# pawanjay176/kzg_rust

Hardware: AMD Instinct MI355X
Metric: blobs/sec on verify_blob_kzg_proof_batch (mainnet 4096, batch=64) (higher is better)
Workload: dtype u32 limbs (29-bit) / 64-bit accumulate, u8 bytes

## Files before the change

__graft_entry__.py:

```python
import os
import subprocess
import sys

ROOT = os.path.dirname(os.path.abspath(__file__))
if ROOT not in sys.path:
    sys.path.insert(0, ROOT)


def build() -> None:
    env = dict(os.environ)
    subprocess.run(["make", "-C", os.path.join(ROOT, "kzg_rust_amd", "csrc"), "-j5"], check=True, env=env)
    subprocess.run(["make", "-C", os.path.join(ROOT, "oracle")], check=True, env=env)
    native = os.path.join(ROOT, "tests", "native")
    subprocess.run(["g++", "-O2", "-shared", "-fPIC", "-o", os.path.join(native, "libhd_probe.so"), os.path.join(native, "hd_probe.cpp")],
                   check=True, env=env)
    subprocess.run(["g++", "-O2", "-shared", "-fPIC", "-o", os.path.join(native, "liblazy_chain_probe.so"), os.path.join(native, "lazy_chain_probe.cpp")],
                   check=True, env=env)
    subprocess.run(["g++", "-O2", "-shared", "-fPIC", "-o", os.path.join(native, "libmont_columns_probe.so"), os.path.join(native, "mont_columns_probe.cpp")],
                   check=True, env=env)
    subprocess.run(["g++", "-std=c++17", "-O2", "-o", os.path.join(native, "cpp_vector_runner"), os.path.join(native, "cpp_vector_runner.cpp"),
                    "-L" + os.path.join(ROOT, "kzg_rust_amd"), "-lkzg355", "-Wl,-rpath," + os.path.join(ROOT, "kzg_rust_amd")], check=True, env=env)
    subprocess.run(["g++", "-std=c++17", "-O2", "-o", os.path.join(native, "cpp_cell_runner"), os.path.join(native, "cpp_cell_runner.cpp"),
                    "-L" + os.path.join(ROOT, "kzg_rust_amd"), "-lkzg355", "-Wl,-rpath," + os.path.join(ROOT, "kzg_rust_amd")], check=True, env=env)
    subprocess.run(["g++", "-std=c++17", "-O2", "-o", os.path.join(native, "cpp_cell_compute_runner"), os.path.join(native, "cpp_cell_compute_runner.cpp"),
                    "-L" + os.path.join(ROOT, "kzg_rust_amd"), "-lkzg355", "-Wl,-rpath," + os.path.join(ROOT, "kzg_rust_amd")], check=True, env=env)
    subprocess.run(["g++", "-std=c++17", "-O2", "-o", os.path.join(native, "cpp_cell_recover_runner"), os.path.join(native, "cpp_cell_recover_runner.cpp"),
                    "-L" + os.path.join(ROOT, "kzg_rust_amd"), "-lkzg355", "-Wl,-rpath," + os.path.join(ROOT, "kzg_rust_amd")], check=True, env=env)
    subprocess.run(["g++", "-std=c++17", "-O2", "-o", os.path.join(native, "cpp_cell_recover_sets_runner"), os.path.join(native, "cpp_cell_recover_sets_runner.cpp"),
                    "-L" + os.path.join(ROOT, "kzg_rust_amd"), "-lkzg355", "-Wl,-rpath," + os.path.join(ROOT, "kzg_rust_amd")], check=True, env=env)
    quad_src, quad_bin = os.path.join(native, "quad_ops_test.hip"), os.path.join(native, "quad_ops_test")
    quad_deps = [quad_src] + [os.path.join(ROOT, "kzg_rust_amd", "csrc", f) for f in ("g1_quad.h", "g1.h", "field.h", "modinv.h", "consts_gen.h")]
    if not os.path.exists(quad_bin) or any(os.path.getmtime(d) > os.path.getmtime(quad_bin) for d in quad_deps):
        subprocess.run(["/opt/rocm/bin/hipcc", "-O3", "-std=c++17", "--offload-arch=gfx950", "-Wno-unused-result", "-o", quad_bin, quad_src], check=True, env=env)
    probe_src, probe_so = os.path.join(native, "gpu_probe.hip"), os.path.join(native, "libgpu_probe.so")
    probe_deps = [probe_src] + [os.path.join(ROOT, "kzg_rust_amd", "csrc", f) for f in ("field.h", "modinv.h", "eval_core.h", "consts_gen.h")]
    if not os.path.exists(probe_so) or any(os.path.getmtime(d) > os.path.getmtime(probe_so) for d in probe_deps):
        subprocess.run(["/opt/rocm/bin/hipcc", "-O3", "-std=c++17", "--offload-arch=gfx950", "-Wno-unused-result", "-shared", "-fPIC", "-o", probe_so, probe_src],
                       check=True, env=env)
    group_src, group_so = os.path.join(native, "gpu_group_probe.hip"), os.path.join(native, "libgpu_group_probe.so")
    group_deps = [group_src] + [os.path.join(ROOT, "kzg_rust_amd", "csrc", f) for f in
                                ("field.h", "modinv.h", "tower.h", "g1.h", "pairing.h", "pairing_coop.h", "pairing_lanes.h", "consts_gen.h")]
    if not os.path.exists(group_so) or any(os.path.getmtime(d) > os.path.getmtime(group_so) for d in group_deps):
        subprocess.run(["/opt/rocm/bin/hipcc", "-O3", "-std=c++17", "--offload-arch=gfx950", "-Wno-unused-result", "-shared", "-fPIC", "-o", group_so, group_src],
                       check=True, env=env)
    import kzg_rust_amd
    from kzg_rust_amd import _lib
    lib = _lib.load()
    for name in _lib.EXPORTED_SYMBOLS:
        getattr(lib, name)
    print("build ok:", lib.kzg355_version().decode())


def smoke() -> None:
    import torch
    assert torch.cuda.is_available(), "smoke() needs a GPU"
    import kzg_rust_amd as kz
    from oracle.oracle import Oracle
    sys.path.insert(0, os.path.join(ROOT, "tests"))
    from synth import random_blob
    golden = os.path.join(ROOT, "tests", "golden")
    g1 = open(os.path.join(golden, "trusted_setup_g1.bin"), "rb").read()
    g2 = open(os.path.join(golden, "trusted_setup_g2.bin"), "rb").read()
    s = kz.Kzg.load_trusted_setup([g1[48 * i:48 * i + 48] for i in range(4096)], [g2[96 * i:96 * i + 96] for i in range(65)])
    o = Oracle()
    os_ = o.load_trusted_setup(g1, g2)
    blobs = [random_blob(1000 + i) for i in range(3)]
    cs = [kz.Kzg.blob_to_kzg_commitment(kz.Blob(b), s) for b in blobs]
    assert [c.to_bytes() for c in cs] == [o.blob_to_kzg_commitment(b, os_) for b in blobs], "commitment mismatch vs oracle"
    ps = [kz.Kzg.compute_blob_kzg_proof(kz.Blob(b), c, s) for b, c in zip(blobs, cs)]
    assert [p.to_bytes() for p in ps] == [o.compute_blob_kzg_proof(b, c.to_bytes(), os_) for b, c in zip(blobs, cs)], "proof mismatch vs oracle"
    ok = kz.Kzg.verify_blob_kzg_proof_batch([kz.Blob(b) for b in blobs], cs, ps, s)
    assert ok is True and o.verify_blob_kzg_proof_batch(blobs, [c.to_bytes() for c in cs], [p.to_bytes() for p in ps], os_) is True
    bad = [ps[1], ps[0], ps[2]]
    assert kz.Kzg.verify_blob_kzg_proof_batch([kz.Blob(b) for b in blobs], cs, bad, s) is False
    s.free()
    o.free_trusted_setup(os_)
    print("smoke ok: commit/prove bit-exact vs oracle, verify batch true/false as expected")


if __name__ == "__main__":
    build()
    if len(sys.argv) > 1 and sys.argv[1] == "smoke":
        smoke()
```

kzg_rust_amd/csrc/eval_core.h:

```cpp
#pragma once
#include "field.h"

namespace kzg {

struct EvalGroup { Fr sa, sb, st; };
constexpr int EVAL_ZPOWERS = 12;
constexpr int EVAL_WAVES = 4;
constexpr int EVAL_TAB_L1 = 0, EVAL_TAB_L2 = 1024, EVAL_TAB_L3 = 1280, EVAL_TAB_L4 = 1344, EVAL_TAB_L5 = 1360, EVAL_TAB_L6 = 1364, EVAL_TAB_GROUPS = 1365;
struct EvalPiece { uint32_t w[4]; };
constexpr int EVAL_TAB_PIECES = ((EVAL_TAB_GROUPS + 63) / 64) * 7 * 64;
KZG_HD constexpr int eval_tab_piece(int e, int q) { return (e / 64) * 7 * 64 + q * 64 + (e % 64); }
KZG_HD void eval_group_pack(EvalPiece p[7], const EvalGroup &g) {
    for (int k = 0; k < 28; k++) p[k / 4].w[k % 4] = k < NFR ? g.sa.l[k] : k < 2 * NFR ? g.sb.l[k - NFR] : k < 3 * NFR ? g.st.l[k - 2 * NFR] : 0u;
}
KZG_HD void eval_group_unpack(EvalGroup &g, const EvalPiece p[7]) {
#pragma unroll
    for (int k = 0; k < 27; k++) (k < NFR ? g.sa.l[k] : k < 2 * NFR ? g.sb.l[k - NFR] : g.st.l[k - 2 * NFR]) = p[k / 4].w[k % 4];
}
KZG_HD constexpr int eval_tab_first(int level) {
    return level == 1 ? EVAL_TAB_L1 : level == 2 ? EVAL_TAB_L2 : level == 3 ? EVAL_TAB_L3 : level == 4 ? EVAL_TAB_L4 : level == 5 ? EVAL_TAB_L5 : EVAL_TAB_L6;
}

template <int K> struct FrMultiple {
    uint32_t l[NFR];
    constexpr FrMultiple() : l{} {
        const uint32_t m[NFR] = FR_MOD_INIT;
        uint64_t c = 0;
        for (int i = 0; i < NFR; i++) { c += (uint64_t)m[i] * (uint32_t)K; l[i] = i < NFR - 1 ? (uint32_t)(c & LMASK) : (uint32_t)c; c >>= LB; }
    }
};
template <int K> KZG_HD void fr_sub_bias(Fr &r, const Fr &a, const Fr &b) {
    constexpr FrMultiple<K> kr;
    int32_t c = 0;
#pragma unroll
    for (int i = 0; i < NFR; i++) {
        const int32_t t = (int32_t)a.l[i] - (int32_t)b.l[i] + (int32_t)kr.l[i] + c;
        if (i < NFR - 1) { c = t >> LB; r.l[i] = (uint32_t)t & LMASK; }
        else r.l[i] = (uint32_t)t;
    }
}

KZG_HD void fr_add_raw(Fr &r, const Fr &a, const Fr &b) {
#pragma unroll
    for (int i = 0; i < NFR; i++) r.l[i] = a.l[i] + b.l[i];
}
template <int K> struct FrMultipleRaw {
    uint32_t l[NFR];
    constexpr FrMultipleRaw() : l{} {
        const FrMultiple<K> n;
        for (int i = 0; i < NFR; i++) l[i] = n.l[i] + (i < NFR - 1 ? (1u << LB) : 0u) - (i > 0 ? 1u : 0u);
    }
};
template <int K> KZG_HD void fr_sub_bias_raw(Fr &r, const Fr &a, const Fr &b) {
    constexpr FrMultipleRaw<K> kr;
#pragma unroll
    for (int i = 0; i < NFR; i++) r.l[i] = a.l[i] - b.l[i] + kr.l[i];
}
KZG_HD void fr_add_sweep(Fr &r, const Fr &a, const Fr &b) {
    uint32_t c = 0;
#pragma unroll
    for (int i = 0; i < NFR; i++) {
        const uint32_t t = a.l[i] + b.l[i] + c;
        if (i < NFR - 1) { c = t >> LB; r.l[i] = t & LMASK; } else r.l[i] = t;
    }
}

template <int K> KZG_HD void eval_node2(Fr &n, const Fr &n0, const Fr &n1, const Fr &zk, const Fr &s) {
    Fr A, B;
    fr_add_raw(A, n0, n1);
    fr_sub_bias_raw<K>(B, n0, n1);
    fr_mul2_lazy(n, A, zk, B, s);
}
KZG_HD void eval_group(Fr &n, const Fr c[4], const Fr &zk, const Fr &zk2, const EvalGroup &g) {
    Fr na, nb;
    eval_node2<2>(na, c[0], c[1], zk, g.sa);
    eval_node2<2>(nb, c[2], c[3], zk, g.sb);
    eval_node2<2>(n, na, nb, zk2, g.st);
}
KZG_HD void eval_group_leaves(Fr &n, Fr &Sp, const uint32_t pw[4][8], const Fr &z, const Fr &z2, const EvalGroup &g) {
    Fr p0, p1, p2, p3, A, B, na, nb, S;
    words_to_limbs<NFR, 8>(p0.l, pw[0]); words_to_limbs<NFR, 8>(p1.l, pw[1]);
    words_to_limbs<NFR, 8>(p2.l, pw[2]); words_to_limbs<NFR, 8>(p3.l, pw[3]);
    fr_add_raw(A, p0, p1); fr_sub_bias_raw<3>(B, p0, p1);
    fr_mul2_lazy(na, A, z, B, g.sa);
    fr_add_raw(S, p2, p3); fr_sub_bias_raw<3>(B, p2, p3);
    fr_mul2_lazy(nb, S, z, B, g.sb);
    fr_add_raw(S, S, A);
    fr_add_sweep(Sp, Sp, S);
    eval_node2<2>(n, na, nb, z2, g.st);
}
KZG_HD void eval_fold(Fr &s) { Fr t; fr_mul_lazy(t, s, fr_one()); s = t; }
KZG_HD void eval_finish(Fr &y, const Fr &ntop, const Fr &Sp, const Fr &z, const Fr &zN) {
    const uint32_t inv4096[NFR] = FR_INV4096_INIT;
    Fr k4096; for (int i = 0; i < NFR; i++) k4096.l[i] = inv4096[i];
    Fr negD, t;
    fr_sub(negD, fr_one(), zN);
    fr_mul2_lazy(t, ntop, z, Sp, negD);
    fr_mul(y, t, k4096);
}

}
```

kzg_rust_amd/csrc/k_verify.hip:

```cpp
#define KZG_FP_MUL_NOINLINE 1
#define KZG_MONT_COLS_FR 1
#include "kernels.h"
#include "sha256_rounds.h"
#include "fr_block.h"

namespace kzg {



constexpr int CH_BLOCKS = 2050;
struct ChallengeReader {
    const uint4 *blob; const uint8_t *cm;
    uint4 line[8];
    uint32_t carry[8];
    __device__ __forceinline__ void prefetch(int b) {
        if (b < 2048 && !(b & 1)) {
            const uint4 *p = blob + 4 * b;
#pragma unroll
            for (int q = 0; q < 8; q++) line[q] = p[q];
        }
    }
    __device__ __forceinline__ void words(uint32_t w[16], int b) {
        if (b == 0) {
            w[0] = 0x4653424cu; w[1] = 0x4f425645u; w[2] = 0x52494659u; w[3] = 0x5f56315fu;
            w[4] = 0; w[5] = 0; w[6] = 0; w[7] = (uint32_t)N_FE;
        } else if (b <= 2048) {
#pragma unroll
            for (int k = 0; k < 8; k++) w[k] = carry[k];
        }
        if (b < 2048) {
            uint4 s0, s1, s2, s3;
            if (b & 1) { s0 = line[4]; s1 = line[5]; s2 = line[6]; s3 = line[7]; }
            else { s0 = line[0]; s1 = line[1]; s2 = line[2]; s3 = line[3]; }
            w[8] = bswap32(s0.x); w[9] = bswap32(s0.y); w[10] = bswap32(s0.z); w[11] = bswap32(s0.w);
            w[12] = bswap32(s1.x); w[13] = bswap32(s1.y); w[14] = bswap32(s1.z); w[15] = bswap32(s1.w);
            carry[0] = bswap32(s2.x); carry[1] = bswap32(s2.y); carry[2] = bswap32(s2.z); carry[3] = bswap32(s2.w);
            carry[4] = bswap32(s3.x); carry[5] = bswap32(s3.y); carry[6] = bswap32(s3.z); carry[7] = bswap32(s3.w);
        } else if (b == 2048) {
            for (int k = 0; k < 8; k++) w[8 + k] = load_be32(cm + 4 * k);
        } else {
            for (int k = 0; k < 4; k++) w[k] = load_be32(cm + 32 + 4 * k);
            w[4] = 0x80000000u;
            for (int k = 5; k < 15; k++) w[k] = 0;
            w[15] = (uint32_t)((32 + BLOB_BYTES + 48) * 8);
        }
    }
};

__device__ __forceinline__ void challenge_finish(const uint32_t hh[8], int i, const uint8_t *cm, const uint8_t *proofs, Fr *z_out, Fr *zpow_out,
        uint8_t *records) {
    const uint32_t dw[8] = {hh[7], hh[6], hh[5], hh[4], hh[3], hh[2], hh[1], hh[0]};
    Fr z; fr_from_words(z, dw);
    z_out[i] = z;
    if (zpow_out) {
        Fr p = z;
#pragma unroll 1
        for (int k = 0; k < EVAL_ZPOWERS; k++) { fr_sqr(p, p); zpow_out[EVAL_ZPOWERS * (size_t)i + k] = p; }
    }
    if (!records) return;
    uint8_t *rec = records + (size_t)RECORD_BYTES * i;
    for (int k = 0; k < 48; k++) rec[k] = cm[k];
    uint8_t zb[32]; fr_to_be32(zb, z);
    for (int k = 0; k < 32; k++) rec[48 + k] = zb[k];
    const uint8_t *pr = proofs + 48 * (size_t)i;
    for (int k = 0; k < 48; k++) rec[112 + k] = pr[k];
}

__global__ void __launch_bounds__(128) k_challenge(const uint8_t *blobs, const uint8_t *commitments, const uint8_t *proofs, int n_total,
                                                    Fr *z_out, Fr *zpow_out, uint8_t *records) {
    __shared__ uint4 wk[2][16][64];
    const int lane = threadIdx.x & 63, role = threadIdx.x >> 6;
    const int i_raw = blockIdx.x * 64 + lane;
    const int i = i_raw < n_total ? i_raw : n_total - 1;
    const uint4 *blob = reinterpret_cast<const uint4 *>(blobs + (size_t)BLOB_BYTES * i);
    const uint8_t *cm = commitments + 48 * (size_t)i;
    static const uint32_t K[64] = {
        0x428a2f98u, 0x71374491u, 0xb5c0fbcfu, 0xe9b5dba5u, 0x3956c25bu, 0x59f111f1u, 0x923f82a4u, 0xab1c5ed5u,
        0xd807aa98u, 0x12835b01u, 0x243185beu, 0x550c7dc3u, 0x72be5d74u, 0x80deb1feu, 0x9bdc06a7u, 0xc19bf174u,
        0xe49b69c1u, 0xefbe4786u, 0x0fc19dc6u, 0x240ca1ccu, 0x2de92c6fu, 0x4a7484aau, 0x5cb0a9dcu, 0x76f988dau,
        0x983e5152u, 0xa831c66du, 0xb00327c8u, 0xbf597fc7u, 0xc6e00bf3u, 0xd5a79147u, 0x06ca6351u, 0x14292967u,
        0x27b70a85u, 0x2e1b2138u, 0x4d2c6dfcu, 0x53380d13u, 0x650a7354u, 0x766a0abbu, 0x81c2c92eu, 0x92722c85u,
        0xa2bfe8a1u, 0xa81a664bu, 0xc24b8b70u, 0xc76c51a3u, 0xd192e819u, 0xd6990624u, 0xf40e3585u, 0x106aa070u,
        0x19a4c116u, 0x1e376c08u, 0x2748774cu, 0x34b0bcb5u, 0x391c0cb3u, 0x4ed8aa4au, 0x5b9cca4fu, 0x682e6ff3u,
        0x748f82eeu, 0x78a5636fu, 0x84c87814u, 0x8cc70208u, 0x90befffau, 0xa4506cebu, 0xbef9a3f7u, 0xc67178f2u};
    ChallengeReader rd; rd.blob = blob; rd.cm = cm;
    auto produce = [&](int b) {
        uint32_t w[16];
        rd.words(w, b);
        rd.prefetch(b + 1);
        uint4 *dst = &wk[b & 1][0][lane];
#pragma unroll
        for (int t = 0; t < 64; t += 4) {
#pragma unroll
            for (int u = 0; u < 4; u++) {
                const int tt = t + u;
                if (tt >= 16) {
                    const uint32_t w15 = w[(tt + 1) & 15], w2 = w[(tt + 14) & 15];
                    const uint32_t s0 = xor3(ror(w15, 7), ror(w15, 18), w15 >> 3);
                    const uint32_t s1 = xor3(ror(w2, 17), ror(w2, 19), w2 >> 10);
                    w[tt & 15] = w[tt & 15] + s0 + w[(tt + 9) & 15] + s1;
                }
            }
            dst[(t >> 2) * 64] = make_uint4(w[t & 15] + K[t], w[(t + 1) & 15] + K[t + 1], w[(t + 2) & 15] + K[t + 2], w[(t + 3) & 15] + K[t + 3]);
        }
    };
    uint32_t h0 = 0x6a09e667u, h1 = 0xbb67ae85u, h2 = 0x3c6ef372u, h3 = 0xa54ff53au, h4 = 0x510e527fu, h5 = 0x9b05688cu, h6 = 0x1f83d9abu, h7 = 0x5be0cd19u;
    if (role == 1) { rd.prefetch(0); produce(0); }
    __syncthreads();
    for (int b = 0; b < CH_BLOCKS; b++) {
        if (role == 0) {
            uint32_t a = h0, bb = h1, c = h2, d = h3, e = h4, f = h5, g = h6, h = h7;
            const uint4 *src = &wk[b & 1][0][lane];
#pragma unroll
            for (int t = 0; t < 64; t += 4) {
                const uint4 q = src[(t >> 2) * 64];
                const uint32_t wv[4] = {q.x, q.y, q.z, q.w};
#pragma unroll
                for (int u = 0; u < 4; u++) {
                    const uint32_t t1 = h + xor3(ror(e, 6), ror(e, 11), ror(e, 25)) + ch3(e, f, g) + wv[u];
                    const uint32_t t2 = xor3(ror(a, 2), ror(a, 13), ror(a, 22)) + maj3(a, bb, c);
                    h = g; g = f; f = e; e = d + t1; d = c; c = bb; bb = a; a = t1 + t2;
                }
            }
            h0 += a; h1 += bb; h2 += c; h3 += d; h4 += e; h5 += f; h6 += g; h7 += h;
        } else if (b + 1 < CH_BLOCKS) {
            produce(b + 1);
        }
        __syncthreads();
    }
    if (role != 0 || i_raw >= n_total) return;
    const uint32_t hh[8] = {h0, h1, h2, h3, h4, h5, h6, h7};
    challenge_finish(hh, i, cm, proofs, z_out, zpow_out, records);
}

constexpr int CH1W_THREADS = 256;
__global__ void __launch_bounds__(CH1W_THREADS) k_challenge_1w(const uint8_t *blobs, const uint8_t *commitments, const uint8_t *proofs, int n_total,
                                                      Fr *z_out, Fr *zpow_out, uint8_t *records) {
    const int i_raw = blockIdx.x * CH1W_THREADS + threadIdx.x;
    const int i = i_raw < n_total ? i_raw : n_total - 1;
    const uint4 *blob = reinterpret_cast<const uint4 *>(blobs + (size_t)BLOB_BYTES * i);
    const uint8_t *cm = commitments + 48 * (size_t)i;
    static const uint32_t K[64] = {
        0x428a2f98u, 0x71374491u, 0xb5c0fbcfu, 0xe9b5dba5u, 0x3956c25bu, 0x59f111f1u, 0x923f82a4u, 0xab1c5ed5u,
        0xd807aa98u, 0x12835b01u, 0x243185beu, 0x550c7dc3u, 0x72be5d74u, 0x80deb1feu, 0x9bdc06a7u, 0xc19bf174u,
        0xe49b69c1u, 0xefbe4786u, 0x0fc19dc6u, 0x240ca1ccu, 0x2de92c6fu, 0x4a7484aau, 0x5cb0a9dcu, 0x76f988dau,
        0x983e5152u, 0xa831c66du, 0xb00327c8u, 0xbf597fc7u, 0xc6e00bf3u, 0xd5a79147u, 0x06ca6351u, 0x14292967u,
        0x27b70a85u, 0x2e1b2138u, 0x4d2c6dfcu, 0x53380d13u, 0x650a7354u, 0x766a0abbu, 0x81c2c92eu, 0x92722c85u,
        0xa2bfe8a1u, 0xa81a664bu, 0xc24b8b70u, 0xc76c51a3u, 0xd192e819u, 0xd6990624u, 0xf40e3585u, 0x106aa070u,
        0x19a4c116u, 0x1e376c08u, 0x2748774cu, 0x34b0bcb5u, 0x391c0cb3u, 0x4ed8aa4au, 0x5b9cca4fu, 0x682e6ff3u,
        0x748f82eeu, 0x78a5636fu, 0x84c87814u, 0x8cc70208u, 0x90befffau, 0xa4506cebu, 0xbef9a3f7u, 0xc67178f2u};
    uint32_t hh[8] = {0x6a09e667u, 0xbb67ae85u, 0x3c6ef372u, 0xa54ff53au, 0x510e527fu, 0x9b05688cu, 0x1f83d9abu, 0x5be0cd19u};
    ChallengeReader rd; rd.blob = blob; rd.cm = cm;
    rd.prefetch(0);
#pragma unroll 1
    for (int b = 0; b < CH_BLOCKS; b++) {
        uint32_t w[16];
        rd.words(w, b);
        rd.prefetch(b + 1);
        uint32_t a = hh[0], bb = hh[1], c = hh[2], d = hh[3], e = hh[4], f = hh[5], g = hh[6], h = hh[7];
#pragma unroll
        for (int t = 0; t < 64; t++) {
            if (t >= 16) {
                const uint32_t w15 = w[(t + 1) & 15], w2 = w[(t + 14) & 15];
                const uint32_t s0 = xor3(ror(w15, 7), ror(w15, 18), w15 >> 3);
                const uint32_t s1 = xor3(ror(w2, 17), ror(w2, 19), w2 >> 10);
                w[t & 15] = w[t & 15] + s0 + w[(t + 9) & 15] + s1;
            }
            const uint32_t t1 = h + xor3(ror(e, 6), ror(e, 11), ror(e, 25)) + ch3(e, f, g) + (w[t & 15] + K[t]);
            const uint32_t t2 = xor3(ror(a, 2), ror(a, 13), ror(a, 22)) + maj3(a, bb, c);
            h = g; g = f; f = e; e = d + t1; d = c; c = bb; bb = a; a = t1 + t2;
        }
        hh[0] += a; hh[1] += bb; hh[2] += c; hh[3] += d; hh[4] += e; hh[5] += f; hh[6] += g; hh[7] += h;
    }
    if (i_raw >= n_total) return;
    challenge_finish(hh, i, cm, proofs, z_out, zpow_out, records);
}

__global__ void __launch_bounds__(64) k_challenge_from_digest(const uint8_t *digests, const uint8_t *commitments, const uint8_t *proofs, int n_total,
                                                              Fr *z_out, Fr *zpow_out, uint8_t *records) {
    const int i = blockIdx.x * 64 + threadIdx.x;
    if (i >= n_total) return;
    uint32_t hh[8];
#pragma unroll
    for (int k = 0; k < 8; k++) hh[k] = load_be32(digests + 32 * (size_t)i + 4 * k);
    challenge_finish(hh, i, commitments + 48 * (size_t)i, proofs, z_out, zpow_out, records);
}

__device__ __forceinline__ void eval_issue_tile_loads(const uint4 *blob_step, uint4 *tile, int lane) {
#pragma unroll
    for (int q = 0; q < 8; q++) {
        const int g = 8 * q + (lane >> 3), s = lane & 7;
        __builtin_amdgcn_global_load_lds((const void __attribute__((address_space(1))) *)(blob_step + 8 * g + (s ^ (g & 7))),
                                         (void __attribute__((address_space(3))) *)(tile + 64 * q), 16, 0, 0);
    }
}
__device__ __forceinline__ void eval_tab_load(EvalPiece p[7], const EvalPiece *tab, int e) {
    const uint4 *src = reinterpret_cast<const uint4 *>(tab);
#pragma unroll
    for (int q = 0; q < 7; q++) { const uint4 v = src[eval_tab_piece(e, q)]; p[q].w[0] = v.x; p[q].w[1] = v.y; p[q].w[2] = v.z; p[q].w[3] = v.w; }
}
__device__ __forceinline__ void eval_park(uint32_t *hx, int entry, const Fr &h) {
#pragma unroll
    for (int k = 0; k < NFR; k++) hx[NFR * entry + k] = h.l[k];
}
__device__ __forceinline__ void eval_children(Fr c[4], const uint32_t *hx, int node) {
    __builtin_amdgcn_fence(__ATOMIC_RELEASE, "workgroup"); __builtin_amdgcn_wave_barrier(); __builtin_amdgcn_fence(__ATOMIC_ACQUIRE, "workgroup");
    const uint4 *src = reinterpret_cast<const uint4 *>(hx + 4 * NFR * node);
    uint32_t w[4 * NFR];
#pragma unroll
    for (int q = 0; q < NFR; q++) { const uint4 v = src[q]; w[4 * q] = v.x; w[4 * q + 1] = v.y; w[4 * q + 2] = v.z; w[4 * q + 3] = v.w; }
#pragma unroll
    for (int e = 0; e < 4; e++)
#pragma unroll
        for (int k = 0; k < NFR; k++) c[e].l[k] = w[NFR * e + k];
    __builtin_amdgcn_fence(__ATOMIC_RELEASE, "workgroup"); __builtin_amdgcn_wave_barrier();
}
__global__ void __launch_bounds__(64 * EVAL_WAVES, 2) k_eval(const uint8_t *blobs, const Fr *z_in, const Fr *zpow, const EvalPiece *tab, int n_total,
                                                          int n_per_group, Fr *y_out, uint8_t *records, int *err) {
    __shared__ uint4 tiles[EVAL_WAVES][512];
    __shared__ __attribute__((aligned(16))) uint32_t hxs[EVAL_WAVES][256 * NFR];
    const int wid = __builtin_amdgcn_readfirstlane((int)(threadIdx.x >> 6)), lane = threadIdx.x & 63;
    const int blob_raw = blockIdx.x * EVAL_WAVES + wid;
    const int blob_i = blob_raw < n_total ? blob_raw : n_total - 1;
    uint4 *tile = tiles[wid];
    uint32_t *hx = hxs[wid];
    const uint4 *blob = reinterpret_cast<const uint4 *>(blobs + (size_t)BLOB_BYTES * blob_i);
    eval_issue_tile_loads(blob, tile, lane);
    const Fr z = z_in[blob_i];
    const Fr *zp = zpow + EVAL_ZPOWERS * (size_t)blob_i;
    const Fr z2 = zp[0];
    __shared__ uint32_t zls[EVAL_WAVES][4 * NFR];
    const uint32_t zl_word = reinterpret_cast<const uint32_t *>(zp + 1)[lane < 4 * NFR ? lane : 0];
    Fr h2[4], Sp = fr_zero();
    bool bad = false;
    constexpr int STEPS = N_FE / 4 / 64;
    EvalPiece g_next[7];
    eval_tab_load(g_next, tab, EVAL_TAB_L1 + lane);
#pragma unroll 1
    for (int it = 0; it < STEPS; it++) {
        __builtin_amdgcn_s_waitcnt(0);
        __builtin_amdgcn_fence(__ATOMIC_ACQUIRE, "workgroup");
        if (it == 0 && lane < 4 * NFR) zls[wid][lane] = zl_word;
        uint4 cur[8];
#pragma unroll
        for (int j = 0; j < 8; j++) cur[j] = tile[8 * lane + (j ^ (lane & 7))];
        EvalGroup g1; eval_group_unpack(g1, g_next);
        __builtin_amdgcn_fence(__ATOMIC_RELEASE, "workgroup"); __builtin_amdgcn_wave_barrier();
        if (it + 1 < STEPS) eval_issue_tile_loads(blob + 512 * (it + 1), tile, lane);
        const int e_l1 = EVAL_TAB_L1 + ((it + 1) & (STEPS - 1)) * 64 + lane, e_l2 = EVAL_TAB_L2 + 64 * (it >> 2) + lane;
        eval_tab_load(g_next, tab, (it & 3) == 3 ? e_l2 : e_l1);
        uint32_t pw[4][8];
#pragma unroll
        for (int e = 0; e < 4; e++) {
            const uint4 a = cur[2 * e], b = cur[2 * e + 1];
            pw[e][7] = bswap32(a.x); pw[e][6] = bswap32(a.y); pw[e][5] = bswap32(a.z); pw[e][4] = bswap32(a.w);
            pw[e][3] = bswap32(b.x); pw[e][2] = bswap32(b.y); pw[e][1] = bswap32(b.z); pw[e][0] = bswap32(b.w);
        }
        const uint32_t top = max(max(pw[0][7], pw[1][7]), max(pw[2][7], pw[3][7]));
        if (top >= FR_MOD_TOP_WORD) {
#pragma unroll 1
            for (int e = 0; e < 4; e++) bad = bad || !fr_words_canonical(pw[e]);
        }
        Fr h;
        eval_group_leaves(h, Sp, pw, z, z2, g1);
        eval_park(hx, 64 * (it & 3) + lane, h);
        if ((it & 3) == 3) {
            Fr c[4];
            eval_children(c, hx, lane);
            EvalGroup g2; eval_group_unpack(g2, g_next);
            eval_tab_load(g_next, tab, it + 1 < STEPS ? e_l1 : EVAL_TAB_L3 + lane);
            Fr z4, z8;
#pragma unroll
            for (int k = 0; k < NFR; k++) { z4.l[k] = zls[wid][k]; z8.l[k] = zls[wid][NFR + k]; }
            Fr r2; eval_group(r2, c, z4, z8, g2);
#pragma unroll
            for (int a = 0; a < 4; a++) if ((it >> 2) == a) h2[a] = r2;
        }
    }
    if (bad && blob_raw < n_total) atomicOr(&err[blob_i / n_per_group], ERR_NONCANONICAL_FR);
    Fr c[4], h;
#pragma unroll
    for (int a = 0; a < 4; a++) eval_park(hx, 64 * a + lane, h2[a]);
    eval_children(c, hx, lane);
    EvalGroup g3; eval_group_unpack(g3, g_next);
    Fr z16, z32;
#pragma unroll
    for (int k = 0; k < NFR; k++) { z16.l[k] = zls[wid][2 * NFR + k]; z32.l[k] = zls[wid][3 * NFR + k]; }
    eval_group(h, c, z16, z32, g3);
    const int b = lane >> 4, u = lane & 15;
    const int mine_raw = blockIdx.x * EVAL_WAVES + b, mine = mine_raw < n_total ? mine_raw : n_total - 1;
    const Fr *zq = zpow + EVAL_ZPOWERS * (size_t)mine;
    Fr zt[7];
#pragma unroll
    for (int k = 0; k < 7; k++) zt[k] = zq[5 + k];
    const Fr zmine = z_in[mine];
    EvalPiece gp4[7], gp5[7], gp6[7];
    eval_tab_load(gp4, tab, EVAL_TAB_L4 + u); eval_tab_load(gp5, tab, EVAL_TAB_L5 + (lane & 3)); eval_tab_load(gp6, tab, EVAL_TAB_L6);
    eval_fold(Sp);
#pragma unroll
    for (int off = 32; off > 0; off >>= 1) { const Fr o = fr_shfl_down(Sp, off); fr_add_lazy(Sp, Sp, o); }
    eval_park(hx, lane, h);
    if (lane == 0) eval_park(hx, 64, Sp);
    __syncthreads();
    if (wid != 0) return;
    Fr Sb;
#pragma unroll
    for (int k = 0; k < NFR; k++) Sb.l[k] = hxs[b][NFR * 64 + k];
    eval_children(c, hxs[b], u);
    EvalGroup gt; eval_group_unpack(gt, gp4);
    eval_group(h, c, zt[0], zt[1], gt);
    uint32_t *hx0 = hxs[0];
    eval_park(hx0, lane, h);
    eval_children(c, hx0, 4 * b + (lane & 3));
    eval_group_unpack(gt, gp5);
    eval_group(h, c, zt[2], zt[3], gt);
    if (u < 4) eval_park(hx0, 4 * b + u, h);
    eval_children(c, hx0, b);
    eval_group_unpack(gt, gp6);
    eval_group(h, c, zt[4], zt[5], gt);
    Fr y; eval_finish(y, h, Sb, zmine, zt[6]);
    if (u == 0 && mine_raw < n_total) {
        if (records) {
            uint32_t yw[8]; limbs_to_words<NFR, 8>(yw, y.l);
            uint8_t *rec = records + (size_t)RECORD_BYTES * mine + 80;
#pragma unroll
            for (int i = 0; i < 8; i++) {
                const uint32_t v = yw[7 - i];
                rec[4 * i] = (uint8_t)(v >> 24); rec[4 * i + 1] = (uint8_t)(v >> 16); rec[4 * i + 2] = (uint8_t)(v >> 8); rec[4 * i + 3] = (uint8_t)v;
            }
        }
        if (y_out) {
            const uint32_t r2[NFR] = FR_R2_INIT;
            Fr R2; for (int i = 0; i < NFR; i++) R2.l[i] = r2[i];
            Fr ym; fr_mul(ym, y, R2);
            y_out[mine] = ym;
        }
    }
}

__global__ void __launch_bounds__(64) k_rhash_lanes(const uint8_t *records, int n, int groups, uint32_t *digests, int n_fe) {
    const int g = blockIdx.x * 64 + threadIdx.x;
    if (g >= groups) return;
    const uint8_t *rec = records + (size_t)RECORD_BYTES * n * g;
    const uint32_t total_words = 8u + 40u * (uint32_t)n;
    const uint32_t nblocks = (total_words * 4u + 9u + 63u) / 64u;
    const uint64_t bits = (uint64_t)total_words * 32u;
    uint32_t hs[8] = {0x6a09e667u, 0xbb67ae85u, 0x3c6ef372u, 0xa54ff53au, 0x510e527fu, 0x9b05688cu, 0x1f83d9abu, 0x5be0cd19u};
#pragma unroll 1
    for (uint32_t b = 0; b < nblocks; b++) {
        uint32_t w[16];
        if (b >= 1u && 16u * b + 16u <= total_words) {
            const uint4 *p = reinterpret_cast<const uint4 *>(rec + 64u * (size_t)b - 32u);
#pragma unroll
            for (int q = 0; q < 4; q++) {
                const uint4 v = p[q];
                w[4 * q] = bswap32(v.x); w[4 * q + 1] = bswap32(v.y); w[4 * q + 2] = bswap32(v.z); w[4 * q + 3] = bswap32(v.w);
            }
        } else {
#pragma unroll
            for (int t = 0; t < 16; t++) {
                const uint32_t idx = 16u * b + (uint32_t)t;
                uint32_t v;
                if (idx < 8u) {
                    const uint32_t hdr[8] = {0x52434b5au, 0x47424154u, 0x43485f5fu, 0x5f56315fu, 0u, (uint32_t)n_fe, 0u, (uint32_t)n};
                    v = hdr[idx];
                } else if (idx < total_words) v = bswap32(reinterpret_cast<const uint32_t *>(rec)[idx - 8u]);
                else if (idx == total_words) v = 0x80000000u;
                else if (idx == 16u * nblocks - 2u) v = (uint32_t)(bits >> 32);
                else if (idx == 16u * nblocks - 1u) v = (uint32_t)bits;
                else v = 0u;
                w[t] = v;
            }
        }
        uint32_t a = hs[0], bb = hs[1], c = hs[2], d = hs[3], e = hs[4], f = hs[5], gg = hs[6], h = hs[7];
#pragma unroll
        for (int t = 0; t < 64; t++) {
            if (t >= 16) {
                const uint32_t w15 = w[(t + 1) & 15], w2 = w[(t + 14) & 15];
                const uint32_t s0 = xor3(ror(w15, 7), ror(w15, 18), w15 >> 3);
                const uint32_t s1 = xor3(ror(w2, 17), ror(w2, 19), w2 >> 10);
                w[t & 15] = w[t & 15] + s0 + w[(t + 9) & 15] + s1;
            }
            const uint32_t t1 = h + xor3(ror(e, 6), ror(e, 11), ror(e, 25)) + ch3(e, f, gg) + w[t & 15] + SHA_K[t];
            const uint32_t t2 = xor3(ror(a, 2), ror(a, 13), ror(a, 22)) + maj3(a, bb, c);
            h = gg; gg = f; f = e; e = d + t1; d = c; c = bb; bb = a; a = t1 + t2;
        }
        hs[0] += a; hs[1] += bb; hs[2] += c; hs[3] += d; hs[4] += e; hs[5] += f; hs[6] += gg; hs[7] += h;
    }
#pragma unroll
    for (int k = 0; k < 8; k++) digests[8 * (size_t)g + k] = hs[7 - k];
}

__global__ void __launch_bounds__(256) k_rpowers(const uint8_t *records, int n, int groups, int check_zy, uint32_t *scal_a, uint32_t *scal_b,
                                                  uint32_t *scal_c, int *err, int n_fe, int have_digest) {
    __shared__ uint32_t wk_all[4][64][64];
    __shared__ uint32_t digest_all[4][8];
    const int wid = threadIdx.x >> 6, lane = threadIdx.x & 63;
    const int g_raw = blockIdx.x * (int)(blockDim.x >> 6) + wid;
    if (g_raw >= groups) return;
    const int g = g_raw;
    const bool live = true;
    uint32_t (*wk)[64] = wk_all[wid];
    uint32_t *digest = digest_all[wid];
    const uint8_t *rec = records + (size_t)RECORD_BYTES * n * g;
    Fr r = fr_one();
    if (n > 1 && have_digest) {
        uint32_t dw[8];
#pragma unroll
        for (int k = 0; k < 8; k++) dw[k] = scal_c[8 * (size_t)g + k];
        fr_from_words(r, dw);
    } else if (n > 1) {
        const uint32_t total_words = 8u + 40u * (uint32_t)n;
        const uint32_t nblocks = (total_words * 4u + 9u + 63u) / 64u;
        const uint64_t bits = (uint64_t)total_words * 32u;
        uint32_t h0 = 0x6a09e667u, h1 = 0xbb67ae85u, h2 = 0x3c6ef372u, h3 = 0xa54ff53au, h4 = 0x510e527fu, h5 = 0x9b05688cu, h6 = 0x1f83d9abu, h7 = 0x5be0cd19u;
        for (uint32_t b0 = 0; b0 < nblocks; b0 += 64) {
            const uint32_t b = b0 + (uint32_t)lane;
            if (b < nblocks) {
                uint32_t w[16];
#pragma unroll
                for (int t = 0; t < 16; t++) {
                    const uint32_t idx = 16u * b + (uint32_t)t;
                    uint32_t v;
                    if (idx < 8u) {
                        const uint32_t hdr[8] = {0x52434b5au, 0x47424154u, 0x43485f5fu, 0x5f56315fu, 0u, (uint32_t)n_fe, 0u, (uint32_t)n};
                        v = hdr[idx];
                    } else if (idx < total_words) v = bswap32(reinterpret_cast<const uint32_t *>(rec)[idx - 8u]);
                    else if (idx == total_words) v = 0x80000000u;
                    else if (idx == 16u * nblocks - 2u) v = (uint32_t)(bits >> 32);
                    else if (idx == 16u * nblocks - 1u) v = (uint32_t)bits;
                    else v = 0u;
                    w[t] = v;
                }
#pragma unroll
                for (int t = 0; t < 64; t++) {
                    if (t >= 16) {
                        const uint32_t w15 = w[(t + 1) & 15], w2 = w[(t + 14) & 15];
                        const uint32_t s0 = xor3(ror(w15, 7), ror(w15, 18), w15 >> 3);
                        const uint32_t s1 = xor3(ror(w2, 17), ror(w2, 19), w2 >> 10);
                        w[t & 15] = w[t & 15] + s0 + w[(t + 9) & 15] + s1;
                    }
                    wk[t][lane] = w[t & 15] + SHA_K[t];
                }
            }
            SHA_WAVE_SYNC();
            if (lane == 0) {
                const uint32_t cnt = nblocks - b0 < 64u ? nblocks - b0 : 64u;
#pragma unroll 1
                for (uint32_t q = 0; q < cnt; q++) {
                    uint32_t a = h0, bb = h1, c = h2, d = h3, e = h4, f = h5, gg = h6, h = h7;
#pragma unroll
                    for (int t = 0; t < 64; t++) {
                        const uint32_t t1 = h + xor3(ror(e, 6), ror(e, 11), ror(e, 25)) + ch3(e, f, gg) + wk[t][q];
                        const uint32_t t2 = xor3(ror(a, 2), ror(a, 13), ror(a, 22)) + maj3(a, bb, c);
                        h = gg; gg = f; f = e; e = d + t1; d = c; c = bb; bb = a; a = t1 + t2;
                    }
                    h0 += a; h1 += bb; h2 += c; h3 += d; h4 += e; h5 += f; h6 += gg; h7 += h;
                }
            }
            SHA_WAVE_SYNC();
        }
        if (lane == 0) { digest[0] = h7; digest[1] = h6; digest[2] = h5; digest[3] = h4; digest[4] = h3; digest[5] = h2; digest[6] = h1; digest[7] = h0; }
        SHA_WAVE_SYNC();
        uint32_t dw[8];
#pragma unroll
        for (int k = 0; k < 8; k++) dw[k] = digest[k];
        fr_from_words(r, dw);
    }
    Fr pw = fr_one(), r64 = r;
#pragma unroll 1
    for (int bit = 5; bit >= 0; bit--) {
        Fr t;
        fr_sqr(pw, pw);
        fr_mul(t, pw, r);
        fr_select(pw, (lane >> bit) & 1, pw, t);
        fr_sqr(r64, r64);
    }
    Fr csum = fr_zero();
    bool bad = false;
#pragma unroll 1
    for (int i = lane; i < n; i += 64) {
        uint32_t zw[8], yw[8];
        be32_to_words(zw, rec + (size_t)RECORD_BYTES * i + 48);
        be32_to_words(yw, rec + (size_t)RECORD_BYTES * i + 80);
        if (check_zy) bad = bad || !fr_words_canonical(zw) || !fr_words_canonical(yw);
        Fr z, y, t; fr_from_words(z, zw); fr_from_words(y, yw);
        uint32_t *pa = scal_a + 8 * ((size_t)g * n + i), *pb = scal_b + 8 * ((size_t)g * n + i);
        uint32_t ow[8];
        fr_to_words(ow, pw); if (live) for (int k = 0; k < 8; k++) pa[k] = ow[k];
        fr_mul(t, pw, z); fr_to_words(ow, t); if (live) for (int k = 0; k < 8; k++) pb[k] = ow[k];
        fr_mul(t, pw, y); fr_add(csum, csum, t);
        fr_mul(pw, pw, r64);
    }
#pragma unroll
    for (int off = 32; off > 0; off >>= 1) { Fr o = fr_shfl_down(csum, off); fr_add(csum, csum, o); }
    if (lane == 0 && live) {
        uint32_t ow[8]; fr_to_words(ow, csum);
        for (int k = 0; k < 8; k++) scal_c[8 * (size_t)g + k] = ow[k];
    }
    if (bad && live) atomicOr(&err[g], ERR_NONCANONICAL_FR);
}

__global__ void __launch_bounds__(64) k_pairing(const PairPt *pair_pts, const LineCoeff *lines, const int *lines_inf, int groups, int *ok) {
    const int g = blockIdx.x * blockDim.x + threadIdx.x;
    if (g >= groups) return;
    G1Affine p1, p2; pairpt_to_affine(p1, pair_pts[2 * (size_t)g]); pairpt_to_affine(p2, pair_pts[2 * (size_t)g + 1]);
    if (lines_inf[2]) p1 = g1a_inf();
    if (lines_inf[0]) p2 = g1a_inf();
    Fp12 f;
    miller_loop_pair(f, lines + 2 * N_LINES, p1, lines, p2);
    ok[g] = final_exp_is_one(f) ? 1 : 0;
}

void launch_challenges(const uint8_t *d_blobs, const uint8_t *d_commitments, const uint8_t *d_proofs, int n_total, Fr *d_z, Fr *d_zpow, uint8_t *d_records,
                       hipStream_t st, int form) {
    if (n_total <= 0) return;
    const int wgs = (n_total + 63) / 64;
    if (form == 2 || (form == 0 && wgs <= 512)) hipLaunchKernelGGL(k_challenge, dim3(wgs), dim3(128), 0, st, d_blobs, d_commitments, d_proofs, n_total, d_z,
            d_zpow, d_records);
    else hipLaunchKernelGGL(k_challenge_1w, dim3((n_total + CH1W_THREADS - 1) / CH1W_THREADS), dim3(CH1W_THREADS), 0, st, d_blobs, d_commitments, d_proofs,
            n_total, d_z, d_zpow, d_records);
}
void launch_challenges_from_digests(const uint8_t *d_digests, const uint8_t *d_commitments, const uint8_t *d_proofs, int n_total, Fr *d_z, Fr *d_zpow,
                                    uint8_t *d_records, hipStream_t st) {
    if (n_total <= 0) return;
    hipLaunchKernelGGL(k_challenge_from_digest, dim3((n_total + 63) / 64), dim3(64), 0, st, d_digests, d_commitments, d_proofs, n_total, d_z, d_zpow,
            d_records);
}
void launch_eval(const uint8_t *d_blobs, const Fr *d_z, const Fr *d_zpow, DeviceTables t, int n_total, int n_per_group, Fr *d_y, uint8_t *d_records, int *d_err,
                 hipStream_t st) {
    if (n_total <= 0) return;
    hipLaunchKernelGGL(k_eval, dim3((n_total + EVAL_WAVES - 1) / EVAL_WAVES), dim3(64 * EVAL_WAVES), 0, st, d_blobs, d_z, d_zpow, t.eval_tab, n_total,
            n_per_group,
                       d_y, d_records, d_err);
}
void launch_rpowers(const uint8_t *d_records, int n_per_group, int groups, int check_zy, uint32_t *d_scal_a, uint32_t *d_scal_b,
                    uint32_t *d_scal_c, int *d_err, hipStream_t st, int n_fe, int lanes_from, int have_digest) {
    if (groups <= 0) return;
    const int wpw = groups > 512 ? 4 : 1;
    const int lanes = (!have_digest && n_per_group > 1 && groups >= lanes_from) ? 1 : 0;
    if (lanes) hipLaunchKernelGGL(k_rhash_lanes, dim3((groups + 63) / 64), dim3(64), 0, st, d_records, n_per_group, groups, d_scal_c, n_fe);
    hipLaunchKernelGGL(k_rpowers, dim3((groups + wpw - 1) / wpw), dim3(64 * wpw), 0, st, d_records, n_per_group, groups, check_zy, d_scal_a, d_scal_b,
            d_scal_c, d_err, n_fe, lanes || have_digest);
}
void launch_pairing_lane(const PairPt *d_pair_pts, DeviceTables t, int groups, int *d_ok, hipStream_t st) {
    if (groups <= 0) return;
    hipLaunchKernelGGL(k_pairing, dim3((groups + 63) / 64), dim3(64), 0, st, d_pair_pts, t.lines, t.lines_inf, groups, d_ok);
}

}
```

Measured before the change: 4.704 million.

## Reorder eval table so level-2 children stay in registers, use buffer loads

Reorders the eval twiddle table so each lane's four level-1 children for a level-2 group come from consecutive iterations. Level-1 results then stay in a register shift array instead of being parked in LDS and shuffled back. The LDS scratch shrinks and the loop is split into nested 4x4 loops. Tile loads move to buffer-resource loads into LDS, tile reads use inline ds_read_b128, and z powers become wave-uniform via readfirstlane. The cost is more live registers (c1 and h2 arrays), with inline asm waits that may serialise work.

```diff
diff --git a/__graft_entry__.py b/__graft_entry__.py
--- a/__graft_entry__.py
+++ b/__graft_entry__.py
@@ -17,6 +17,8 @@
     subprocess.run(["g++", "-O2", "-shared", "-fPIC", "-o", os.path.join(native, "liblazy_chain_probe.so"), os.path.join(native, "lazy_chain_probe.cpp")],
                    check=True, env=env)
     subprocess.run(["g++", "-O2", "-shared", "-fPIC", "-o", os.path.join(native, "libmont_columns_probe.so"), os.path.join(native, "mont_columns_probe.cpp")],
+                   check=True, env=env)
+    subprocess.run(["g++", "-O2", "-shared", "-fPIC", "-o", os.path.join(native, "libeval_tab_probe.so"), os.path.join(native, "eval_tab_probe.cpp")],
                    check=True, env=env)
     subprocess.run(["g++", "-std=c++17", "-O2", "-o", os.path.join(native, "cpp_vector_runner"), os.path.join(native, "cpp_vector_runner.cpp"),
                     "-L" + os.path.join(ROOT, "kzg_rust_amd"), "-lkzg355", "-Wl,-rpath," + os.path.join(ROOT, "kzg_rust_amd")], check=True, env=env)
diff --git a/kzg_rust_amd/csrc/eval_core.h b/kzg_rust_amd/csrc/eval_core.h
--- a/kzg_rust_amd/csrc/eval_core.h
+++ b/kzg_rust_amd/csrc/eval_core.h
@@ -9,7 +9,12 @@
 constexpr int EVAL_TAB_L1 = 0, EVAL_TAB_L2 = 1024, EVAL_TAB_L3 = 1280, EVAL_TAB_L4 = 1344, EVAL_TAB_L5 = 1360, EVAL_TAB_L6 = 1364, EVAL_TAB_GROUPS = 1365;
 struct EvalPiece { uint32_t w[4]; };
 constexpr int EVAL_TAB_PIECES = ((EVAL_TAB_GROUPS + 63) / 64) * 7 * 64;
-KZG_HD constexpr int eval_tab_piece(int e, int q) { return (e / 64) * 7 * 64 + q * 64 + (e % 64); }
+constexpr int EVAL_TAB_ROW_L1 = EVAL_TAB_L1 / 64, EVAL_TAB_ROW_L2 = EVAL_TAB_L2 / 64, EVAL_TAB_ROW_L3 = EVAL_TAB_L3 / 64;
+KZG_HD constexpr int eval_tab_slot(int e) {
+    return e < EVAL_TAB_L2 ? EVAL_TAB_L1 + 64 * (e & 15) + (e >> 4) : e < EVAL_TAB_L3 ? EVAL_TAB_L2 + 64 * ((e - EVAL_TAB_L2) & 3) + ((e - EVAL_TAB_L2) >> 2) : e;
+}
+KZG_HD constexpr int eval_tab_row_piece(int row, int col, int q) { return (row * 7 + q) * 64 + col; }
+KZG_HD constexpr int eval_tab_piece(int e, int q) { return eval_tab_row_piece(eval_tab_slot(e) / 64, eval_tab_slot(e) % 64, q); }
 KZG_HD void eval_group_pack(EvalPiece p[7], const EvalGroup &g) {
     for (int k = 0; k < 28; k++) p[k / 4].w[k % 4] = k < NFR ? g.sa.l[k] : k < 2 * NFR ? g.sb.l[k - NFR] : k < 3 * NFR ? g.st.l[k - 2 * NFR] : 0u;
 }
diff --git a/kzg_rust_amd/csrc/k_verify.hip b/kzg_rust_amd/csrc/k_verify.hip
--- a/kzg_rust_amd/csrc/k_verify.hip
+++ b/kzg_rust_amd/csrc/k_verify.hip
@@ -186,18 +186,17 @@
     challenge_finish(hh, i, commitments + 48 * (size_t)i, proofs, z_out, zpow_out, records);
 }
 
-__device__ __forceinline__ void eval_issue_tile_loads(const uint4 *blob_step, uint4 *tile, int lane) {
+__device__ __forceinline__ void eval_issue_tile_loads(__amdgpu_buffer_rsrc_t blob, int it, uint4 *tile, int lane) {
 #pragma unroll
     for (int q = 0; q < 8; q++) {
         const int g = 8 * q + (lane >> 3), s = lane & 7;
-        __builtin_amdgcn_global_load_lds((const void __attribute__((address_space(1))) *)(blob_step + 8 * g + (s ^ (g & 7))),
-                                         (void __attribute__((address_space(3))) *)(tile + 64 * q), 16, 0, 0);
-    }
-}
-__device__ __forceinline__ void eval_tab_load(EvalPiece p[7], const EvalPiece *tab, int e) {
+        __builtin_amdgcn_raw_ptr_buffer_load_lds(blob, (void __attribute__((address_space(3))) *)(tile + 64 * q), 16, 2048 * g + 16 * (s ^ (g & 7)), 128 * it, 0, 0);
+    }
+}
+__device__ __forceinline__ void eval_tab_load(EvalPiece p[7], const EvalPiece *tab, int row, int col) {
     const uint4 *src = reinterpret_cast<const uint4 *>(tab);
 #pragma unroll
-    for (int q = 0; q < 7; q++) { const uint4 v = src[eval_tab_piece(e, q)]; p[q].w[0] = v.x; p[q].w[1] = v.y; p[q].w[2] = v.z; p[q].w[3] = v.w; }
+    for (int q = 0; q < 7; q++) { const uint4 v = src[eval_tab_row_piece(row, col, q)]; p[q].w[0] = v.x; p[q].w[1] = v.y; p[q].w[2] = v.z; p[q].w[3] = v.w; }
 }
 __device__ __forceinline__ void eval_park(uint32_t *hx, int entry, const Fr &h) {
 #pragma unroll
@@ -215,78 +214,88 @@
         for (int k = 0; k < NFR; k++) c[e].l[k] = w[NFR * e + k];
     __builtin_amdgcn_fence(__ATOMIC_RELEASE, "workgroup"); __builtin_amdgcn_wave_barrier();
 }
+__device__ __forceinline__ void eval_group_take(EvalGroup &g, const EvalPiece p[7]) {
+    EvalPiece t[7];
+#pragma unroll
+    for (int k = 0; k < 28; k++) asm volatile("v_mov_b32 %0, %1" : "=v"(t[k / 4].w[k % 4]) : "v"(p[k / 4].w[k % 4]));
+    eval_group_unpack(g, t);
+}
+typedef uint32_t EvalWords4 __attribute__((ext_vector_type(4)));
+__device__ __forceinline__ void eval_tile_read(uint4 cur[8], const uint4 *tile, int lane) {
+    const uint32_t base = (uint32_t)(uintptr_t)(const __attribute__((address_space(3))) uint4 *)tile + 128u * (uint32_t)lane;
+    uint32_t at[8]; EvalWords4 v[8];
+#pragma unroll
+    for (int j = 0; j < 8; j++) at[j] = base + 16u * (uint32_t)(j ^ (lane & 7));
+    asm volatile("ds_read_b128 %0, %8\n\tds_read_b128 %1, %9\n\tds_read_b128 %2, %10\n\tds_read_b128 %3, %11\n\t"
+                 "ds_read_b128 %4, %12\n\tds_read_b128 %5, %13\n\tds_read_b128 %6, %14\n\tds_read_b128 %7, %15\n\ts_waitcnt lgkmcnt(0)"
+                 : "=&v"(v[0]), "=&v"(v[1]), "=&v"(v[2]), "=&v"(v[3]), "=&v"(v[4]), "=&v"(v[5]), "=&v"(v[6]), "=&v"(v[7])
+                 : "v"(at[0]), "v"(at[1]), "v"(at[2]), "v"(at[3]), "v"(at[4]), "v"(at[5]), "v"(at[6]), "v"(at[7]) : "memory");
+#pragma unroll
+    for (int j = 0; j < 8; j++) cur[j] = make_uint4(v[j].x, v[j].y, v[j].z, v[j].w);
+}
+__device__ __forceinline__ Fr eval_uniform(const Fr &v) {
+    Fr r;
+#pragma unroll
+    for (int k = 0; k < NFR; k++) r.l[k] = __builtin_amdgcn_readfirstlane(v.l[k]);
+    return r;
+}
+constexpr int EVAL_HX_ENTRIES = 68;
 __global__ void __launch_bounds__(64 * EVAL_WAVES, 2) k_eval(const uint8_t *blobs, const Fr *z_in, const Fr *zpow, const EvalPiece *tab, int n_total,
                                                           int n_per_group, Fr *y_out, uint8_t *records, int *err) {
-    __shared__ uint4 tiles[EVAL_WAVES][512];
-    __shared__ __attribute__((aligned(16))) uint32_t hxs[EVAL_WAVES][256 * NFR];
+    constexpr int TILES_U4 = EVAL_WAVES * 512, HX_WORDS = EVAL_HX_ENTRIES * NFR;
+    __shared__ uint4 lds[TILES_U4 + EVAL_WAVES * HX_WORDS / 4];
+    uint32_t *hxs = reinterpret_cast<uint32_t *>(lds + TILES_U4);
     const int wid = __builtin_amdgcn_readfirstlane((int)(threadIdx.x >> 6)), lane = threadIdx.x & 63;
     const int blob_raw = blockIdx.x * EVAL_WAVES + wid;
     const int blob_i = blob_raw < n_total ? blob_raw : n_total - 1;
-    uint4 *tile = tiles[wid];
-    uint32_t *hx = hxs[wid];
-    const uint4 *blob = reinterpret_cast<const uint4 *>(blobs + (size_t)BLOB_BYTES * blob_i);
-    eval_issue_tile_loads(blob, tile, lane);
-    const Fr z = z_in[blob_i];
+    uint4 *tile = lds + 512 * wid;
+    uint32_t *hx = hxs + HX_WORDS * wid;
+    const __amdgpu_buffer_rsrc_t blob = __builtin_amdgcn_make_buffer_rsrc(const_cast<uint8_t *>(blobs + (size_t)BLOB_BYTES * blob_i), 0, BLOB_BYTES, 0x00020000);
+    constexpr int STEPS = N_FE / 4 / 64;
+    EvalPiece g_next[7], g_l2[7];
+    eval_tab_load(g_next, tab, EVAL_TAB_ROW_L1, lane);
+    eval_issue_tile_loads(blob, 0, tile, lane);
     const Fr *zp = zpow + EVAL_ZPOWERS * (size_t)blob_i;
-    const Fr z2 = zp[0];
-    __shared__ uint32_t zls[EVAL_WAVES][4 * NFR];
-    const uint32_t zl_word = reinterpret_cast<const uint32_t *>(zp + 1)[lane < 4 * NFR ? lane : 0];
-    Fr h2[4], Sp = fr_zero();
+    const Fr z = eval_uniform(z_in[blob_i]), z2 = eval_uniform(zp[0]), z4 = eval_uniform(zp[1]), z8 = eval_uniform(zp[2]);
+    Fr c1[4], h2[4], Sp = fr_zero();
+#pragma unroll
+    for (int a = 0; a < 4; a++) c1[a] = h2[a] = fr_zero();
     bool bad = false;
-    constexpr int STEPS = N_FE / 4 / 64;
-    EvalPiece g_next[7];
-    eval_tab_load(g_next, tab, EVAL_TAB_L1 + lane);
-#pragma unroll 1
-    for (int it = 0; it < STEPS; it++) {
-        __builtin_amdgcn_s_waitcnt(0);
-        __builtin_amdgcn_fence(__ATOMIC_ACQUIRE, "workgroup");
-        if (it == 0 && lane < 4 * NFR) zls[wid][lane] = zl_word;
-        uint4 cur[8];
-#pragma unroll
-        for (int j = 0; j < 8; j++) cur[j] = tile[8 * lane + (j ^ (lane & 7))];
-        EvalGroup g1; eval_group_unpack(g1, g_next);
-        __builtin_amdgcn_fence(__ATOMIC_RELEASE, "workgroup"); __builtin_amdgcn_wave_barrier();
-        if (it + 1 < STEPS) eval_issue_tile_loads(blob + 512 * (it + 1), tile, lane);
-        const int e_l1 = EVAL_TAB_L1 + ((it + 1) & (STEPS - 1)) * 64 + lane, e_l2 = EVAL_TAB_L2 + 64 * (it >> 2) + lane;
-        eval_tab_load(g_next, tab, (it & 3) == 3 ? e_l2 : e_l1);
-        uint32_t pw[4][8];
-#pragma unroll
-        for (int e = 0; e < 4; e++) {
-            const uint4 a = cur[2 * e], b = cur[2 * e + 1];
-            pw[e][7] = bswap32(a.x); pw[e][6] = bswap32(a.y); pw[e][5] = bswap32(a.z); pw[e][4] = bswap32(a.w);
-            pw[e][3] = bswap32(b.x); pw[e][2] = bswap32(b.y); pw[e][1] = bswap32(b.z); pw[e][0] = bswap32(b.w);
-        }
-        const uint32_t top = max(max(pw[0][7], pw[1][7]), max(pw[2][7], pw[3][7]));
-        if (top >= FR_MOD_TOP_WORD) {
-#pragma unroll 1
-            for (int e = 0; e < 4; e++) bad = bad || !fr_words_canonical(pw[e]);
-        }
-        Fr h;
-        eval_group_leaves(h, Sp, pw, z, z2, g1);
-        eval_park(hx, 64 * (it & 3) + lane, h);
-        if ((it & 3) == 3) {
-            Fr c[4];
-            eval_children(c, hx, lane);
-            EvalGroup g2; eval_group_unpack(g2, g_next);
-            eval_tab_load(g_next, tab, it + 1 < STEPS ? e_l1 : EVAL_TAB_L3 + lane);
-            Fr z4, z8;
-#pragma unroll
-            for (int k = 0; k < NFR; k++) { z4.l[k] = zls[wid][k]; z8.l[k] = zls[wid][NFR + k]; }
-            Fr r2; eval_group(r2, c, z4, z8, g2);
-#pragma unroll
-            for (int a = 0; a < 4; a++) if ((it >> 2) == a) h2[a] = r2;
-        }
+#pragma unroll 1
+    for (int a = 0; a < 4; a++) {
+#pragma unroll 1
+        for (int k = 0; k < 4; k++) {
+            const int it = 4 * a + k;
+            __builtin_amdgcn_s_waitcnt(0);
+            EvalGroup g1; eval_group_take(g1, g_next);
+            eval_tab_load(g_next, tab, it + 1 < STEPS ? EVAL_TAB_ROW_L1 + it + 1 : EVAL_TAB_ROW_L3, lane);
+            if (k == 3) eval_tab_load(g_l2, tab, EVAL_TAB_ROW_L2 + a, lane);
+            uint4 cur[8];
+            eval_tile_read(cur, tile, lane);
+            eval_issue_tile_loads(blob, min(it + 1, STEPS - 1), tile, lane);
+            uint32_t pw[4][8];
+#pragma unroll
+            for (int e = 0; e < 4; e++) {
+                const uint4 hi = cur[2 * e], lo = cur[2 * e + 1];
+                pw[e][7] = bswap32(hi.x); pw[e][6] = bswap32(hi.y); pw[e][5] = bswap32(hi.z); pw[e][4] = bswap32(hi.w);
+                pw[e][3] = bswap32(lo.x); pw[e][2] = bswap32(lo.y); pw[e][1] = bswap32(lo.z); pw[e][0] = bswap32(lo.w);
+            }
+            const uint32_t top = max(max(pw[0][7], pw[1][7]), max(pw[2][7], pw[3][7]));
+            if (top >= FR_MOD_TOP_WORD) {
+#pragma unroll 1
+                for (int e = 0; e < 4; e++) bad = bad || !fr_words_canonical(pw[e]);
+            }
+            c1[0] = c1[1]; c1[1] = c1[2]; c1[2] = c1[3];
+            eval_group_leaves(c1[3], Sp, pw, z, z2, g1);
+        }
+        EvalGroup g2; eval_group_unpack(g2, g_l2);
+        h2[0] = h2[1]; h2[1] = h2[2]; h2[2] = h2[3];
+        eval_group(h2[3], c1, z4, z8, g2);
     }
     if (bad && blob_raw < n_total) atomicOr(&err[blob_i / n_per_group], ERR_NONCANONICAL_FR);
     Fr c[4], h;
-#pragma unroll
-    for (int a = 0; a < 4; a++) eval_park(hx, 64 * a + lane, h2[a]);
-    eval_children(c, hx, lane);
     EvalGroup g3; eval_group_unpack(g3, g_next);
-    Fr z16, z32;
-#pragma unroll
-    for (int k = 0; k < NFR; k++) { z16.l[k] = zls[wid][2 * NFR + k]; z32.l[k] = zls[wid][3 * NFR + k]; }
-    eval_group(h, c, z16, z32, g3);
+    eval_group(h, h2, zp[3], zp[4], g3);
     const int b = lane >> 4, u = lane & 15;
     const int mine_raw = blockIdx.x * EVAL_WAVES + b, mine = mine_raw < n_total ? mine_raw : n_total - 1;
     const Fr *zq = zpow + EVAL_ZPOWERS * (size_t)mine;
@@ -295,7 +304,8 @@
     for (int k = 0; k < 7; k++) zt[k] = zq[5 + k];
     const Fr zmine = z_in[mine];
     EvalPiece gp4[7], gp5[7], gp6[7];
-    eval_tab_load(gp4, tab, EVAL_TAB_L4 + u); eval_tab_load(gp5, tab, EVAL_TAB_L5 + (lane & 3)); eval_tab_load(gp6, tab, EVAL_TAB_L6);
+    eval_tab_load(gp4, tab, (EVAL_TAB_L4 + u) / 64, (EVAL_TAB_L4 + u) % 64); eval_tab_load(gp5, tab, EVAL_TAB_L5 / 64, EVAL_TAB_L5 % 64 + (lane & 3));
+    eval_tab_load(gp6, tab, EVAL_TAB_L6 / 64, EVAL_TAB_L6 % 64);
     eval_fold(Sp);
 #pragma unroll
     for (int off = 32; off > 0; off >>= 1) { const Fr o = fr_shfl_down(Sp, off); fr_add_lazy(Sp, Sp, o); }
@@ -305,11 +315,11 @@
     if (wid != 0) return;
     Fr Sb;
 #pragma unroll
-    for (int k = 0; k < NFR; k++) Sb.l[k] = hxs[b][NFR * 64 + k];
-    eval_children(c, hxs[b], u);
+    for (int k = 0; k < NFR; k++) Sb.l[k] = hxs[HX_WORDS * b + NFR * 64 + k];
+    eval_children(c, hxs + HX_WORDS * b, u);
     EvalGroup gt; eval_group_unpack(gt, gp4);
     eval_group(h, c, zt[0], zt[1], gt);
-    uint32_t *hx0 = hxs[0];
+    uint32_t *hx0 = hxs;
     eval_park(hx0, lane, h);
     eval_children(c, hx0, 4 * b + (lane & 3));
     eval_group_unpack(gt, gp5);
```

Result: no change. 4.700 million (-0.1%).
